# seryrzu/centroFlye

Measured on AMD Instinct MI355X. Metric: long-read bases/sec through rare-k-mer recruit+distance, higher is better.
Workload: dtype u8 bases -> u64 k-mers / u32 indices (integer only)

## Files before the change

### centroflye_amd/csrc/hip/cf_dist.hip

```cpp
#include "cf_common.h"

#include <cstdlib>

void cf_free_edges(cf_ctx* c);
int cf_refresh_unique_count(cf_ctx* ctx);

#define DIST_STAGE_CAP 1024
#define DIST_STACK 112
#define DIST_UNROLL 4
#define DIST_ITEM (64u * DIST_UNROLL)
#define DIST_BM_BITS 65536u
#define DIST_HOT_CAP 2048u
#define DIST_MEMBER_KEYS 8
#define DIST_EDGE_CHUNK 8192ull
#define DIST_OVQ 160u
#define DIST_LDS_HEAD (DIST_BM_BITS / 8 + 128)
#define DIST_CNT_MASK 0x7FFFFFu
#define DIST_SEL_BIT (1ull << 23)

#ifndef cf_ballot
__device__ __forceinline__ unsigned long long cf_ballot(bool p) { return __builtin_amdgcn_ballot_w64(p); }
#endif

struct alignas(16) cf_dist_rec { uint32_t e0; uint32_t len; uint32_t ig; uint32_t nu; };
// ... 138 lines not shown
    const unsigned long long lt = (1ull << lane) - 1ull;
    for (int64_t s0 = wave * (64 * kRounds); s0 < n_kmers; s0 += n_waves * (64 * kRounds)) {
        uint32_t takes = 0, total = 0;
#pragma unroll
        for (int r = 0; r < kRounds; ++r) {
            const int64_t a = s0 + (int64_t)r * 64 + lane;
            const bool take = a < n_kmers && (a % n_parts) == part && pcnt[a] > 0;
            takes |= (uint32_t)take << r;
            total += (uint32_t)__popcll(cf_ballot(take));
        }
        if (total == 0u) continue;
        unsigned long long base = 0;
        if (lane == 0) base = atomicAdd(n_out, (unsigned long long)total);
        base = __shfl(base, 0);
#pragma unroll
        for (int r = 0; r < kRounds; ++r) {
            const bool take = (takes >> r) & 1u;
            const unsigned long long m = cf_ballot(take);
            if (take) {
                const int64_t a = s0 + (int64_t)r * 64 + lane;
                unsigned long long h = 0;
                if (hashed) {
                    const int64_t p0 = post_ptr[a], p1 = post_ptr[a + 1];
                    if (by_second) h = (unsigned long long)(uint32_t)post[p1 - p0 > 1 ? p0 + 1 : p0] & ((1ull << hb) - 1ull);
                    else {
                    h = (unsigned long long)(p1 - p0);
                    for (int64_t p = p0; p < p1; ++p) { h = (h ^ (unsigned long long)(uint32_t)post[p]) * 0x9E3779B97F4A7C15ull; h ^= h >> 29; }
                    h = (h * 0xBF58476D1CE4E5B9ull) >> (64 - hb);
                    }
                }
                keys[base + (unsigned long long)__popcll(m & lt)] = ((unsigned long long)first_unit[a] << (ab + hb)) | (h << ab) | (unsigned long long)a;
            }
            base += (unsigned long long)__popcll(m);
        }
    }
}
__global__ void __launch_bounds__(256)
cf_order_extract_kernel(const unsigned long long* __restrict__ keys, int64_t n, int ab, int32_t* __restrict__ order) {
    const int64_t stride = (int64_t)gridDim.x * blockDim.x;
    for (int64_t i = (int64_t)blockIdx.x * blockDim.x + threadIdx.x; i < n; i += stride) order[i] = (int32_t)(keys[i] & ((1ull << ab) - 1ull));
}

#define DIST_CLASS_CAP 255u
__device__ __forceinline__ bool cf_same_postings(const int64_t* __restrict__ post_ptr, const int32_t* __restrict__ post, uint32_t x, uint32_t y) {
    const int64_t x0 = post_ptr[x], x1 = post_ptr[x + 1], y0 = post_ptr[y], y1 = post_ptr[y + 1];
    if (x1 - x0 != y1 - y0) return false;
    for (int64_t i = 0; i < x1 - x0; ++i) if (post[x0 + i] != post[y0 + i]) return false;
    return true;
}
__global__ void __launch_bounds__(256)
cf_class_mark_kernel(const unsigned long long* __restrict__ keys, int64_t n, int ab, const int64_t* __restrict__ post_ptr, const int32_t* __restrict__ post,
                     const unsigned long long* __restrict__ not_a_set, uint32_t* __restrict__ flags) {
    const unsigned long long rank_mask = (1ull << ab) - 1ull;
    const bool off = *not_a_set != 0ull;
    auto continues = [&](int64_t i) -> bool {
        const unsigned long long k0 = keys[i - 1], k1 = keys[i];
        return (k0 >> ab) == (k1 >> ab) && cf_same_postings(post_ptr, post, (uint32_t)(k0 & rank_mask), (uint32_t)(k1 & rank_mask));
    };
    const int64_t stride = (int64_t)gridDim.x * blockDim.x;
    for (int64_t i = (int64_t)blockIdx.x * blockDim.x + threadIdx.x; i < n; i += stride) {
        if (off) { flags[i] = 1u; continue; }
        if (i > 0 && continues(i)) continue;
        flags[i] = 1u;
        uint32_t run = 1;
        for (int64_t j = i + 1; j < n && continues(j); ++j) {
            if (run == DIST_CLASS_CAP) { flags[j] = 1u; run = 0; }
            ++run;
        }
    }
}
__global__ void __launch_bounds__(256)
cf_class_first_kernel(const uint32_t* __restrict__ flags, const int64_t* __restrict__ cidx, int64_t n, int64_t n_classes, uint32_t* __restrict__ cfirst) {
    const int64_t stride = (int64_t)gridDim.x * blockDim.x;
    for (int64_t i = (int64_t)blockIdx.x * blockDim.x + threadIdx.x; i < n; i += stride) {
        if (flags[i]) cfirst[cidx[i]] = (uint32_t)i;
        if (i == 0) cfirst[n_classes] = (uint32_t)n;
    }
}

#define DIST_GROUP_MAX 32u
__device__ __forceinline__ unsigned long long cf_readlane64(unsigned long long v, int l) {
    return ((unsigned long long)(uint32_t)__builtin_amdgcn_readlane((int)(uint32_t)(v >> 32), l) << 32) | (unsigned long long)(uint32_t)__builtin_amdgcn_readlane((int)(uint32_t)v, l);
}
__global__ void __launch_bounds__(256)
cf_group_mark_kernel(const unsigned long long* __restrict__ keys, int64_t n, int kb, int ab, const int64_t* __restrict__ post_ptr, const int32_t* __restrict__ post,
                     const unsigned long long* __restrict__ not_a_set, uint32_t cap, uint32_t* __restrict__ flags, uint32_t* __restrict__ member_mask, uint32_t* __restrict__ new_mask) {
    const uint32_t lane = threadIdx.x & 63u;
    const int64_t wave = ((int64_t)blockIdx.x * blockDim.x + threadIdx.x) >> 6, n_waves = ((int64_t)gridDim.x * blockDim.x) >> 6;
    const unsigned long long rank_mask = (1ull << ab) - 1ull;
    const bool off = *not_a_set != 0ull;
    for (int64_t c0 = wave * 64; c0 < n; c0 += n_waves * 64) {
        int64_t wb = c0, w_p0 = 0;
        unsigned long long w_fu = ~0ull;
        uint32_t w_len = 0;
        auto load_window = [&](int64_t b) {
            wb = b; w_fu = ~0ull; w_p0 = 0; w_len = 0;
            const int64_t i = b + (int64_t)lane;
            if (i < n) { const unsigned long long k = keys[i]; const uint32_t x = (uint32_t)(k & rank_mask); w_fu = k >> kb; w_p0 = post_ptr[x]; w_len = (uint32_t)(post_ptr[x + 1] - w_p0); }
        };
        load_window(c0);
        const int64_t i_me = c0 + (int64_t)lane;
        if (off) { if (i_me < n) { flags[i_me] = 1u; member_mask[i_me] = 0u; new_mask[i_me] = 0u; } continue; }
        bool head = i_me < n;
        if (head && i_me > 0) head = (keys[i_me - 1] >> kb) != w_fu;
        unsigned long long hm = cf_ballot(head);
        while (hm) {
            const int s = __ffsll((long long)hm) - 1;
            hm &= hm - 1ull;
            if (wb != c0) load_window(c0);
            const unsigned long long fu = cf_readlane64(w_fu, s);
            uint32_t un = 0xFFFFFFFFu, nu = 0, members = 0;
            for (int64_t j = c0 + s; j < n; ++j) {
                if (j - wb == 64) load_window(j);
                const int sl = (int)(j - wb);
                if (cf_readlane64(w_fu, sl) != fu) break;
                const int64_t p0 = (int64_t)cf_readlane64((unsigned long long)w_p0, sl);
                const uint32_t len = (uint32_t)__builtin_amdgcn_readlane((int)w_len, sl);
                if (len > cap) {
                    if (lane == 0u) { flags[j] = 1u; member_mask[j] = 0u; new_mask[j] = 0u; }
                    nu = 0; members = 0;
                    continue;
                }
                const uint32_t L = lane < len ? (uint32_t)post[p0 + lane] : 0xFFFFFFFFu;
                uint32_t mask = 0;
                unsigned long long found = 0;
                for (uint32_t i = 0; i < nu; ++i) {
                    const unsigned long long h = cf_ballot(L == (uint32_t)__builtin_amdgcn_readlane((int)un, (int)i));
                    if (h) { mask |= 1u << i; found |= h; }
                }
                const unsigned long long mine = cf_ballot(lane < len);
                unsigned long long nm = mine & ~found;
                const bool start = members == 0u || members == DIST_CLASS_CAP || nu + (uint32_t)__popcll(nm) > cap;
                if (start) { nu = 0; members = 0; mask = 0; nm = mine; }
                const uint32_t fresh = (uint32_t)nm;
                while (nm) {
                    const int t = __ffsll((long long)nm) - 1;
                    nm &= nm - 1ull;
                    const uint32_t x = (uint32_t)__builtin_amdgcn_readlane((int)L, t);
                    if (lane == nu) un = x;
                    mask |= 1u << nu;
                    ++nu;
                }
                ++members;
                if (lane == 0u) { if (start) flags[j] = 1u; member_mask[j] = mask; new_mask[j] = fresh; }
            }
        }
    }
}
__global__ void __launch_bounds__(256)
cf_group_fill_kernel(const int32_t* __restrict__ order, const uint32_t* __restrict__ gfirst, int64_t n_groups, const int64_t* __restrict__ post_ptr, const int32_t* __restrict__ post,
                     const unsigned long long* __restrict__ not_a_set, uint32_t cap, const uint32_t* __restrict__ new_mask, const uint32_t* __restrict__ member_mask,
                     int32_t* __restrict__ upost, uint32_t* __restrict__ ulen, unsigned long long* __restrict__ diag, unsigned long long* __restrict__ err) {
    const bool off = *not_a_set != 0ull;
    unsigned long long dg_u = 0, dg_c = 0;
    const int64_t stride = (int64_t)gridDim.x * blockDim.x;
    for (int64_t g = (int64_t)blockIdx.x * blockDim.x + threadIdx.x; g < n_groups; g += stride) {
        const uint32_t f = gfirst[g], e = gfirst[g + 1];
        bool counting = off;
        if (e - f == 1u) { const int32_t x = order[f]; counting = counting || (uint32_t)(post_ptr[x + 1] - post_ptr[x]) > cap; }
        uint32_t k = 0;
        if (!counting)
            for (uint32_t j = f; j < e; ++j) {
                uint32_t nm = new_mask[j];
                if (!nm) continue;
                const int64_t p0 = post_ptr[order[j]];
                while (nm) {
                    const int t = __ffs((int)nm) - 1;
                    nm &= nm - 1u;
                    if (k < DIST_GROUP_MAX) upost[(size_t)DIST_GROUP_MAX * (size_t)g + k] = post[p0 + t];
                    ++k;
                }
            }
        if (k > DIST_GROUP_MAX) { atomicOr(err, 4ull); k = DIST_GROUP_MAX; }
        ulen[g] = counting ? 0x80000000u : k;
        dg_u += k;
#if defined(CF_DIST_DIAG_COUNT)
        for (uint32_t j = f; j < e; ++j) {
            bool seen = false;
            for (uint32_t q = f; q < j && !seen; ++q) seen = member_mask[q] == member_mask[j];
            dg_c += (unsigned long long)!seen;
        }
#endif
    }
#if defined(CF_DIST_DIAG_COUNT)
    for (int d = 32; d >= 1; d >>= 1) { dg_u += __shfl_down(dg_u, (unsigned)d); dg_c += __shfl_down(dg_c, (unsigned)d); }
    if ((threadIdx.x & 63) == 0 && dg_c) { atomicAdd(diag, dg_u); atomicAdd(diag + 1, dg_c); }
#else
    (void)diag; (void)dg_u; (void)dg_c; (void)member_mask;
#endif
}
__global__ void __launch_bounds__(256)
cf_member_emissions_kernel(const int32_t* __restrict__ order, int64_t n_order, const int64_t* __restrict__ post_ptr, const int32_t* __restrict__ post,
                           const cf_dist_rec* __restrict__ urange, const int32_t* __restrict__ rend, int32_t min_d, int32_t max_d,
                           unsigned long long* __restrict__ entries_out, unsigned long long* __restrict__ self_out) {
    unsigned long long ent = 0, self = 0;
    const int64_t stride = (int64_t)gridDim.x * blockDim.x;
    for (int64_t i = (int64_t)blockIdx.x * blockDim.x + threadIdx.x; i < n_order; i += stride) {
        const int32_t x = order[i];
        const int64_t p0 = post_ptr[x], p1 = post_ptr[x + 1];
        int32_t u = p0 < p1 ? post[p0] : 0;
        for (int64_t p = p0; p < p1; ++p) {
            ent += urange[u].len;
            const int32_t u_next = p + 1 < p1 ? post[p + 1] : 0x7FFFFFFF;
            if (u_next < rend[u]) {
                for (int64_t q = p + 1; q < p1; ++q) {
                    const int32_t v = post[q];
                    if (v >= rend[u] || v - u > max_d) break;
                    self += (unsigned long long)(v - u >= min_d);
                }
            }
            u = u_next;
        }
    }
    for (int d = 32; d >= 1; d >>= 1) { ent += __shfl_down(ent, (unsigned)d); self += __shfl_down(self, (unsigned)d); }
    if ((threadIdx.x & 63) == 0) {
        if (ent) atomicAdd(entries_out, ent);
        if (self) atomicAdd(self_out, self);
    }
}

struct alignas(8) cf_dist_item { uint32_t e, m; };
#ifndef CF_DIST_ITEMS_BLOCKED
#define CF_DIST_ITEMS_BLOCKED 0
#endif
struct alignas(16) cf_dist_head { uint32_t a, n_items; unsigned long long ibase; uint32_t n_entries, n_useful, n_members, first_member; };

struct cf_dist_args {
    const int64_t* post_ptr;
    const int32_t* post;
    const int64_t* cloud_ptr;
    const int32_t* entries;
    const int32_t* unit_rend;
    const int32_t* unit_rbeg;
    const cf_dist_rec* urange;
    const uint16_t* entry_i;
    const uint8_t* entry_i8;
    uint32_t reg_shift;
    const uint32_t* packed;
    int64_t n_kmers;
    int32_t part, n_parts;
    int32_t min_d, max_d;
    uint32_t min_cov;
    double thr;
    uint32_t thr_num, thr_den;
    int32_t slots;
    uint32_t fill_limit;
    uint32_t est_limit;
    int32_t sketch;
    uint32_t sk_counters, sk_shift, sk_mask;
    uint32_t sk_fbits, sk_fsh, sk_wshift, sk_fmask, sk_guard, sk_bytes;
    const cf_dist_head* heads;
    const cf_dist_item* items;
    uint32_t stage_cap;
    uint32_t filter_once;
    uint32_t hot_cap;
    uint32_t hot_entries;
    uint32_t* edges;
    unsigned long long edge_cap;
    const uint32_t* member_mask;
    const int32_t* order;
    int64_t n_order;
    unsigned long long edge_chunk;
    unsigned long long* holes;
    unsigned long long* counters;
    uint32_t* unique_bits;
};

typedef uint32_t cf_raw4 __attribute__((ext_vector_type(4)));
struct __attribute__((packed, aligned(4))) cf_run4 { uint32_t x, y, z, w; };
__device__ __forceinline__ void cf_load_packed4(const cf_dist_args& A, uint32_t s_e, uint32_t l4, uint32_t& x, uint32_t& y, uint32_t& z, uint32_t& w) {
#if !defined(CF_NO_BUFFER_LOAD)
    const __amdgpu_buffer_rsrc_t rs = __builtin_amdgcn_make_buffer_rsrc((void*)A.packed, 0, (int)0xFFFFFFFFu, 0x00020000);
    const cf_raw4 v = __builtin_amdgcn_raw_buffer_load_b128(rs, (int)(l4 * 4u), (int)(s_e << 2), 0);
    x = v.x; y = v.y; z = v.z; w = v.w;
#else
    const uint32_t* p = A.packed + s_e;
    const cf_run4 r = *(const cf_run4*)(p + l4);
    x = r.x; y = r.y; z = r.z; w = r.w;
#endif
}

struct alignas(16) cf_u64x2 { unsigned long long x, y; };
struct alignas(16) cf_u32x4 { uint32_t x, y, z, w; };

template <int DB>
struct cf_tab_wide_t {
    static constexpr uint32_t kCntBits = 31 - DB, kCntMask = (1u << kCntBits) - 1u, kDMask = (1u << DB) - 1u, kDShift = 32 - DB;
    static constexpr uint32_t kSlotBytes = 8, kPerBucket = 4;
    static constexpr bool kMaskTab = false;
    struct bucket { cf_u64x2 lo, hi; };
    struct raw { uint32_t b, i; };
    typedef unsigned long long qitem;
    static __device__ __forceinline__ qitem q_make(uint32_t b, uint32_t dd, uint32_t bk) { return ((unsigned long long)b << 32) | ((unsigned long long)dd << kDShift) | bk; }
    static __device__ __forceinline__ void q_take(qitem q, uint32_t n_buckets, uint32_t& b, uint32_t& dd, uint32_t& bk) { b = (uint32_t)(q >> 32); dd = ((uint32_t)q >> kDShift) & kDMask; bk = (uint32_t)q & ((1u << kDShift) - 1u); }
    __device__ __forceinline__ qitem q_of(uint32_t b, uint32_t dd, uint32_t n_buckets) const { return q_make(b, dd, home(hash(b), n_buckets)); }
    static __device__ __forceinline__ uint32_t next(uint32_t bk, uint32_t, uint32_t n_buckets) { return bk + 1 == n_buckets ? 0u : bk + 1; }
    __device__ __forceinline__ void configure(const cf_dist_args&, uint32_t) {}
    unsigned long long* tab;
    __device__ __forceinline__ void init(unsigned char* lds, uint32_t) { tab = (unsigned long long*)lds; }
    __device__ __forceinline__ void clear(uint32_t slots, uint32_t t, uint32_t nt) const {
        const cf_u64x2 z{0ull, 0ull};
// ... 1959 lines not shown
        unsigned long long partner_units = 0;
        for (int64_t r = min_n; r < max_n; ++r) {
            const int64_t nu = v_h_unit_ptr[(size_t)r + 1] - v_h_unit_ptr[(size_t)r];
            const int64_t span = (int64_t)max_d - min_d_eff + 1;
            if (nu <= min_d_eff || span <= 0) continue;
            const int64_t full = std::max<int64_t>(0, nu - max_d);
            const int64_t tail = nu - min_d_eff - full;
            partner_units += (unsigned long long)(full * span) + (unsigned long long)(tail > 0 ? tail * (tail + 1) / 2 : 0);
        }
        const double cloud = (double)(e1 - e0) / (double)(u1 - u0), post_per_unit = (double)n_post / (double)(u1 - u0);
        per_first = (double)partner_units * cloud * post_per_unit / (double)std::max<int64_t>(1, (K - part + n_parts - 1) / n_parts);
    }
    const bool groups = groups_fit && per_first <= 32768.0;
    const uint32_t slot_bytes = groups ? cf_tab_mask<8>::kSlotBytes : (narrow || region) ? cf_tab_narrow::kSlotBytes : cf_tab_wide::kSlotBytes;
    int wgs = ctx->dist_wgs, block = ctx->dist_block;
    if (wgs == 0) wgs = (block > 512 || per_first > 32768.0) ? 1 : 2;
    if (block == 0) block = wgs == 1 ? 1024 : 512;
    const size_t qitem_bytes = narrow ? sizeof(cf_tab_narrow::qitem) : sizeof(cf_tab_wide::qitem);
    const size_t lds_fixed = DIST_LDS_HEAD + (size_t)(2 * DIST_STACK) * 4 + DIST_STAGE_CAP * 2 + 16 + (size_t)(block / 64) * (DIST_QSTRIDE + DIST_OVQ) * qitem_bytes + DIST_HOT_CAP * 2
                             + (groups ? (((size_t)(block / 64) * (DIST_QSTRIDE + DIST_OVQ) + 15) & ~(size_t)15) : 0);
    const int64_t budget8 = ((int64_t)160 * 1024 / wgs - (int64_t)lds_fixed) / 8;
    if (budget8 < 256) return cf_fail(ctx, -22, "cf_dist_edges: dist_wgs leaves no LDS for the table");
    if (ctx->dist_slots > budget8) return cf_fail(ctx, -22, "cf_dist_edges: dist_slots does not fit the 160 KiB LDS next to the work lists");
    const int64_t slots8 = ctx->dist_slots ? ctx->dist_slots : budget8;
    A.slots = (int32_t)((slots8 * 8 / slot_bytes) & ~(region ? (int64_t)(32 << reg_shift) - 1 : 7ll));
    if (groups) {
        A.slots = (int32_t)((slots8 * 8 / cf_tab_mask<8>::kSlotBytes) & ~7ll);
        while (A.slots > 8 && (int64_t)A.slots * cf_tab_mask<8>::kSlotBytes + cf_tab_mask<8>::extra_bytes((uint32_t)A.slots) > slots8 * 8) A.slots -= 8;
    }
    const size_t tab_extra = groups ? cf_tab_mask<8>::extra_bytes((uint32_t)A.slots) : 0;
    if (A.slots >= 0xFFFF) return cf_fail(ctx, -22, "cf_dist_edges: more than 65534 table slots (16-bit slot indices; 0xFFFF marks an unused entry of the hot list)");
    A.fill_limit = (uint32_t)((int64_t)A.slots * ctx->dist_fill_pct / 100);
    {
        const int64_t slack = (int64_t)(block / 64) * 2 * 128;
        if (slack * 4 <= (int64_t)A.slots) A.fill_limit = (uint32_t)std::min<int64_t>(A.fill_limit, (int64_t)A.slots - slack);
    }
    A.est_limit = (uint32_t)((int64_t)A.fill_limit * 100 / ctx->dist_est_pct);
    A.counters = d_cnt; A.unique_bits = ctx->d_unique_bits;
    const size_t lds = (size_t)A.slots * slot_bytes + tab_extra + lds_fixed;
    A.sketch = (ctx->dist_sketch && min_cov >= 2 && min_cov <= 200) ? 1 : 0;
    A.sk_shift = 32; A.sk_counters = 1;
    const size_t sk_room = (size_t)A.slots * slot_bytes + DIST_STAGE_CAP * 2 + 16 + (size_t)(block / 64) * (DIST_QSTRIDE + DIST_OVQ) * qitem_bytes + 2 * DIST_STACK * 4 + DIST_HOT_CAP * 2;
    while (A.sk_shift > 8 && (size_t)A.sk_counters * 2 <= sk_room) { A.sk_counters *= 2; --A.sk_shift; }
    if (A.sk_counters < 16) A.sketch = 0;
    A.sk_bytes = A.sk_counters;
    const bool sk4 = A.sketch && min_cov <= 9 && ctx->dist_sketch_bits != 8 && A.sk_shift > 9;
    if (sk4) { A.sk_counters *= 2; --A.sk_shift; A.sk_fbits = 4; A.sk_fsh = 2; A.sk_wshift = 3; A.sk_fmask = 15; A.sk_guard = 12; }
    else { A.sk_fbits = 8; A.sk_fsh = 3; A.sk_wshift = 2; A.sk_fmask = 255; A.sk_guard = 0x7FFFFFFFu; }
    A.sk_mask = A.sk_counters - 1u;
    const int per_cu = std::max(1, std::min((int)((160 * 1024) / lds), 2048 / block));
    const int64_t n_a_alloc = (K > part) ? (K - part + n_parts - 1) / n_parts : 0;
    CF_TRY(tmp.get(&d_okeys, (size_t)n_a_alloc, "order keys"));
    CF_TRY(tmp.get(&d_otmp, (size_t)n_a_alloc, "order scratch"));
    CF_TRY(tmp.get(&d_order, (size_t)n_a_alloc, "order"));
    int ab = 1, ub = 1;
    while (ab < 32 && ((int64_t)1 << ab) < K) ++ab;
    while (ub < 32 && ((int64_t)1 << ub) < std::max<int64_t>(U, 2)) ++ub;
    const bool classes = ctx->dist_classes && by_sort;
    const int hb = classes ? std::min(ctx->dist_class_bits, 64 - ab - ub) : 0;
    int64_t n_heads = 0;
    uint32_t *d_cflag = nullptr, *d_cfirst = nullptr, *d_ulen = nullptr, *d_mmask = nullptr, *d_newm = nullptr;
    int32_t* d_upost = nullptr;
    if (K) {
        hipLaunchKernelGGL(cf_order_keys_kernel, dim3((unsigned)cf_grid_for(K, 256, max_blocks)), dim3(256), 0, ctx->stream,
                           (const uint32_t*)d_pcnt, (const uint32_t*)d_first, K, (int)part, (int)n_parts, ab, d_okeys, d_cnt + 6,
                           hb, (const int64_t*)d_post_ptr, (const int32_t*)d_post, (const unsigned long long*)(d_cnt + 144), groups ? 1 : 0);
        unsigned long long h_n = 0;
        CF_HIP(hipMemcpy(&h_n, d_cnt + 6, 8, hipMemcpyDeviceToHost));
        n_order = (int64_t)h_n;
        CF_TRY(cf_radix_sort_u64(ctx, d_okeys, d_otmp, n_order, ab + hb + ub));
        if (n_order)
            hipLaunchKernelGGL(cf_order_extract_kernel, dim3((unsigned)cf_grid_for(n_order, 256, max_blocks)), dim3(256), 0, ctx->stream,
                               (const unsigned long long*)d_okeys, n_order, ab, d_order);
    }
    n_heads = n_order;
    if (classes && n_order) {
        const unsigned g_cls = (unsigned)cf_grid_for(n_order, 256, max_blocks);
        int64_t* d_cidx = (int64_t*)d_otmp;
        CF_TRY(tmp.get(&d_cflag, (size_t)n_order + 1, "class flags"));
        CF_TRY(tmp.get(&d_cfirst, (size_t)n_order + 1, "class starts"));
        CF_HIP(hipMemsetAsync(d_cflag, 0, (size_t)(n_order + 1) * 4, ctx->stream));
        if (groups) { CF_TRY(tmp.get(&d_mmask, (size_t)n_order + 1, "member masks")); CF_TRY(tmp.get(&d_newm, (size_t)n_order + 1, "members' new postings")); }
        if (groups)
            hipLaunchKernelGGL(cf_group_mark_kernel, dim3(g_cls), dim3(256), 0, ctx->stream, (const unsigned long long*)d_okeys, n_order, ab + hb, ab,
                               (const int64_t*)d_post_ptr, (const int32_t*)d_post, (const unsigned long long*)(d_cnt + 144), (uint32_t)ctx->dist_group_cap, d_cflag, d_mmask, d_newm);
        else
        hipLaunchKernelGGL(cf_class_mark_kernel, dim3(g_cls), dim3(256), 0, ctx->stream, (const unsigned long long*)d_okeys, n_order, ab,
                           (const int64_t*)d_post_ptr, (const int32_t*)d_post, (const unsigned long long*)(d_cnt + 144), d_cflag);
        CF_TRY(cf_scan_exclusive_u32_to_i64(ctx, d_cflag, d_cidx, n_order, &n_heads));
        hipLaunchKernelGGL(cf_class_first_kernel, dim3(g_cls), dim3(256), 0, ctx->stream, (const uint32_t*)d_cflag, (const int64_t*)d_cidx, n_order, n_heads, d_cfirst);
        if (groups) {
            CF_TRY(tmp.get(&d_upost, (size_t)n_heads * DIST_GROUP_MAX + 1, "group unions"));
            CF_TRY(tmp.get(&d_ulen, (size_t)n_heads + 1, "group union sizes"));
            hipLaunchKernelGGL(cf_group_fill_kernel, dim3((unsigned)cf_grid_for(n_heads, 256, max_blocks)), dim3(256), 0, ctx->stream, (const int32_t*)d_order, (const uint32_t*)d_cfirst, n_heads,
                               (const int64_t*)d_post_ptr, (const int32_t*)d_post, (const unsigned long long*)(d_cnt + 144), (uint32_t)ctx->dist_group_cap, (const uint32_t*)d_newm, (const uint32_t*)d_mmask,
                               d_upost, d_ulen, d_cnt + 148, d_cnt + 4);
            hipLaunchKernelGGL(cf_member_emissions_kernel, dim3(g_cls), dim3(256), 0, ctx->stream, (const int32_t*)d_order, n_order, (const int64_t*)d_post_ptr, (const int32_t*)d_post,
                               (const cf_dist_rec*)d_urange, (const int32_t*)d_rend, min_d_eff, max_d, d_cnt + 1, d_cnt + 3);
        }
        CF_KERNEL_CHECK("the class kernels");
    }
    A.order = d_order; A.n_order = n_heads; A.member_mask = d_mmask;
    if (n_heads) {
        const uint32_t nw = (uint32_t)block / 64u;
        const int g_items = cf_grid_for(n_heads * 16, 256, max_blocks);
        CF_TRY(tmp.get(&d_icnt, (size_t)n_heads + 1, "item counts"));
        CF_TRY(tmp.get(&d_ialloc, (size_t)n_heads + 1, "item slots"));
        CF_TRY(tmp.get(&d_ibase, (size_t)n_heads + 1, "item bases"));
        CF_TRY(tmp.get(&d_heads, (size_t)n_heads, "first k-mer heads"));
        hipLaunchKernelGGL(groups ? cf_items_count_kernel<true> : cf_items_count_kernel<false>, dim3((unsigned)g_items), dim3(256), 0, ctx->stream, (const int32_t*)d_order, n_heads, (const int64_t*)d_post_ptr,
                           (const int32_t*)d_post, (const cf_dist_rec*)d_urange, (const int32_t*)d_rbeg, min_d_eff, max_d, nw, by_sort ? 1 : 0, d_icnt, d_ialloc, d_cnt + 3,
                           (const uint32_t*)d_cfirst, (const int32_t*)d_upost, (const uint32_t*)d_ulen);
        CF_TRY(cf_scan_exclusive_u32_to_i64(ctx, d_ialloc, d_ibase, n_heads, &n_item_slots));
        CF_TRY(tmp.get(&d_items, (size_t)n_item_slots + 64, "item records"));
        hipLaunchKernelGGL(groups ? cf_items_fill_kernel<true> : cf_items_fill_kernel<false>, dim3((unsigned)g_items), dim3(256), 0, ctx->stream, (const int32_t*)d_order, n_heads, (const int64_t*)d_post_ptr,
                           (const int32_t*)d_post, (const cf_dist_rec*)d_urange, nw, (const uint32_t*)d_icnt, (const int64_t*)d_ibase, d_heads, d_items,
                           v_cloud_ptr, region26 ? 1 : 0, U, min_d_eff, max_d, min_cov, (ctx->dist_sketch_tail && A.sketch) ? 1 : 0,
                           (const unsigned long long*)(d_cnt + 144), d_cnt + 145, (const uint32_t*)d_cfirst, (const int32_t*)d_upost, (const uint32_t*)d_ulen);
    }
    A.heads = d_heads; A.items = d_items;
    const int64_t n_a = n_heads;
    const int grid = (int)std::max<int64_t>(1, std::min<int64_t>(n_a, (int64_t)std::max(1, ctx->n_cu) * per_cu));
    CF_KERNEL_CHECK("the work-list kernels");
    CF_HIP(hipEventRecord(ctx->ev2, ctx->stream));
#define CF_DIST_KERN(CLS) (region26 ? cf_dist_kernel<cf_tab_region26, CLS> : region ? cf_dist_kernel<cf_tab_region, CLS> : !narrow ? (wide16 ? cf_dist_kernel<cf_tab_wide16, CLS> : cf_dist_kernel<cf_tab_wide, CLS>) \
                               : narrow_db == 8 ? cf_dist_kernel<cf_tab_narrow_t<8>, CLS> : narrow_db == 7 ? cf_dist_kernel<cf_tab_narrow_t<7>, CLS>                                               \
                               : narrow_db == 6 ? cf_dist_kernel<cf_tab_narrow_t<6>, CLS> : cf_dist_kernel<cf_tab_narrow_t<5>, CLS>)
    void (*kern)(cf_dist_args) = classes ? CF_DIST_KERN(true) : CF_DIST_KERN(false);
#if CF_DIST_HAS_GROUPS
    if (groups) kern = narrow_db == 8 ? cf_dist_kernel<cf_tab_mask<8>, true> : narrow_db == 7 ? cf_dist_kernel<cf_tab_mask<7>, true> : narrow_db == 6 ? cf_dist_kernel<cf_tab_mask<6>, true> : cf_dist_kernel<cf_tab_mask<5>, true>;
#endif
#undef CF_DIST_KERN
    CF_HIP(hipFuncSetAttribute((const void*)kern, hipFuncAttributeMaxDynamicSharedMemorySize, (int)lds));
    {
        A.edge_chunk = ctx->dist_edge_chunk > 0 ? (unsigned long long)ctx->dist_edge_chunk : DIST_EDGE_CHUNK;
        const int64_t rows = edge_cap > 0 ? edge_cap + (int64_t)grid * (int64_t)A.edge_chunk : 0;
        CF_TRY(cf_alloc_t(ctx, &ctx->d_edges, (size_t)rows * 4, "edges"));
        ctx->edge_cap = rows;
        A.edges = ctx->d_edges; A.edge_cap = (unsigned long long)rows;
    }
    CF_TRY(tmp.get(&d_holes, 2 * ((size_t)grid + 1), "edge holes"));
    A.holes = d_holes;
    CF_HIP(hipMemsetAsync(d_cnt + 6, 0, 16, ctx->stream));
    if (n_a > 0 && max_d >= min_d_eff && n_post > 0) {
        hipLaunchKernelGGL(kern, dim3((unsigned)grid), dim3((unsigned)block), lds, ctx->stream, A);
        CF_KERNEL_CHECK("cf_dist_kernel");
    }
    CF_HIP(hipEventRecord(ctx->ev3, ctx->stream));
    CF_HIP(hipMemcpyAsync(h_cnt, d_cnt, 64, hipMemcpyDeviceToHost, ctx->stream));
    CF_HIP(hipEventRecord(ctx->ev1, ctx->stream));
    CF_HIP(hipEventSynchronize(ctx->ev1));
#if defined(CF_DIST_DIAG_COUNT)
    {
        unsigned long long st[8];
        if (hipMemcpy(st, d_cnt + 8, 64, hipMemcpyDeviceToHost) == hipSuccess)
            std::fprintf(stderr, "[cf_dist diag] parked-insert loop trips=%llu overflow calls=%llu parked inserts run=%llu drains=%llu inserts drained=%llu cycles(sum over waves): parked runs=%llu drains=%llu table sweeps=%llu; waves=%d passes=%llu\n", st[0], st[1], st[2], st[3], st[4], st[5], st[6], st[7], grid * (block / 64), h_cnt[5]);
        unsigned long long su[4], up[2] = {0, 0};
        const bool have_up = groups && hipMemcpy(up, d_cnt + 148, 16, hipMemcpyDeviceToHost) == hipSuccess;
        if (hipMemcpy(su, d_cnt + 144, 32, hipMemcpyDeviceToHost) == hipSuccess)
            std::fprintf(stderr, "[cf_dist diag] sketch items=%llu of items=%llu (rows are sets=%d) classes=%lld members=%lld entries swept=%llu of %llu per member\n", su[1], su[2], su[0] ? 0 : 1, have_up ? (long long)up[1] : (long long)n_heads, (long long)n_order, su[3], h_cnt[1]);
        unsigned long long mf[5];
        if (hipMemcpy(mf, d_cnt + 152, 40, hipMemcpyDeviceToHost) == hipSuccess)
            std::fprintf(stderr, "[cf_dist diag] member filter: n_hot=%llu n_hot x members=%llu eval_slot calls with total_of=%llu buckets read in total_of=%llu slots with more keys than registers=%llu\n", mf[0], mf[1], mf[2], mf[3], mf[4]);
        if (have_up)
            std::fprintf(stderr, "[cf_dist diag] groups=%lld members=%lld union postings=%llu slots=%d split groups=%llu\n", (long long)n_heads, (long long)n_order, up[0], (int)A.slots, h_cnt[2]);
    }
#endif
#if defined(CF_DIST_STAMPS)
    {
        unsigned long long st[8];
        if (hipMemcpy(st, d_cnt + 8, 64, hipMemcpyDeviceToHost) == hipSuccess)
            std::fprintf(stderr, "[cf_dist stamps] pop=%llu prologue=%llu sketch=%llu clear=%llu stream=%llu filter=%llu write=%llu sweep_end_wait=%llu (shader cycles summed over %d workgroups; passes=%llu)\n",
                         st[0], st[1], st[6], st[2], st[3], st[4], st[5], st[7], grid, h_cnt[5]);
    }
#endif
    if (h_cnt[4] & 4ull) return cf_fail(ctx, -5, "cf_dist_edges: internal error, a group's union has more postings than its mask has bits");
    if (h_cnt[4] & 2ull) return cf_fail(ctx, -5, "cf_dist_edges: the kernel's dynamic LDS does not begin at address 0");
    if (h_cnt[4]) return cf_fail(ctx, -34, "cf_dist_edges: (b,d) table could not be partitioned far enough");
    {
        const unsigned long long a_cap = std::min<unsigned long long>(h_cnt[0], A.edge_cap);
        std::vector<unsigned long long> hh(2 * (size_t)h_cnt[7]);
// ... 59 lines not shown
```

Before: 4.847 billion.

## Fuse member emissions into group-walk kernel with LDS-staged postings and team fill

Replaces the group mark kernel with a walk kernel that stages each window's posting lists into per-wave LDS rows using 8-lane teams. The entry and self-distance counts come from those staged rows in the same pass, so the separate member-emissions kernel and its second read of postings are gone. The member loop now reads postings from LDS with a prefetch, and per-member outputs are buffered in lanes and stored coalesced. The fill kernel moves from one thread per group to 8-lane teams with a prefix-sum scatter. In exchange it adds LDS use that may lower occupancy, more register pressure, and a more complex control flow with correctness risk (caps clamped to 32).

```diff
diff --git a/centroflye_amd/csrc/hip/cf_dist.hip b/centroflye_amd/csrc/hip/cf_dist.hip
--- a/centroflye_amd/csrc/hip/cf_dist.hip
+++ b/centroflye_amd/csrc/hip/cf_dist.hip
@@ -244,23 +244,121 @@
 __device__ __forceinline__ unsigned long long cf_readlane64(unsigned long long v, int l) {
     return ((unsigned long long)(uint32_t)__builtin_amdgcn_readlane((int)(uint32_t)(v >> 32), l) << 32) | (unsigned long long)(uint32_t)__builtin_amdgcn_readlane((int)(uint32_t)v, l);
 }
+#define DIST_WALK_ROW 33u
+#define DIST_WALK_LDS(block) ((size_t)((block) / 64) * 64 * DIST_WALK_ROW * 4)
 __global__ void __launch_bounds__(256)
-cf_group_mark_kernel(const unsigned long long* __restrict__ keys, int64_t n, int kb, int ab, const int64_t* __restrict__ post_ptr, const int32_t* __restrict__ post,
-                     const unsigned long long* __restrict__ not_a_set, uint32_t cap, uint32_t* __restrict__ flags, uint32_t* __restrict__ member_mask, uint32_t* __restrict__ new_mask) {
+cf_group_walk_kernel(const unsigned long long* __restrict__ keys, int64_t n, int kb, int ab, const int64_t* __restrict__ post_ptr, const int32_t* __restrict__ post,
+                     const unsigned long long* __restrict__ not_a_set, uint32_t cap, const cf_dist_rec* __restrict__ urange, const int32_t* __restrict__ rend, int32_t min_d, int32_t max_d,
+                     uint32_t* __restrict__ flags, uint32_t* __restrict__ member_mask, uint32_t* __restrict__ new_mask,
+                     unsigned long long* __restrict__ entries_out, unsigned long long* __restrict__ self_out) {
     const uint32_t lane = threadIdx.x & 63u;
+    uint32_t* const rows = (uint32_t*)cf_lds + (size_t)(threadIdx.x >> 6) * (64u * DIST_WALK_ROW);
     const int64_t wave = ((int64_t)blockIdx.x * blockDim.x + threadIdx.x) >> 6, n_waves = ((int64_t)gridDim.x * blockDim.x) >> 6;
     const unsigned long long rank_mask = (1ull << ab) - 1ull;
     const bool off = *not_a_set != 0ull;
+    if (cap > DIST_GROUP_MAX) cap = DIST_GROUP_MAX;
+    unsigned long long ent = 0, self = 0;
     for (int64_t c0 = wave * 64; c0 < n; c0 += n_waves * 64) {
         int64_t wb = c0, w_p0 = 0;
         unsigned long long w_fu = ~0ull;
-        uint32_t w_len = 0;
-        auto load_window = [&](int64_t b) {
+        uint32_t w_len = 0, o_mask = 0, o_new = 0;
+        bool o_start = false, o_done = false;
+        auto flush = [&]() {
+            if (o_done) { const int64_t i = wb + (int64_t)lane; flags[i] = o_start ? 1u : 0u; member_mask[i] = o_mask; new_mask[i] = o_new; }
+            o_done = false;
+        };
+        auto load_window = [&](int64_t b, bool all, bool own, unsigned long long fu) {
+            flush();
             wb = b; w_fu = ~0ull; w_p0 = 0; w_len = 0;
             const int64_t i = b + (int64_t)lane;
-            if (i < n) { const unsigned long long k = keys[i]; const uint32_t x = (uint32_t)(k & rank_mask); w_fu = k >> kb; w_p0 = post_ptr[x]; w_len = (uint32_t)(post_ptr[x + 1] - w_p0); }
+            if (i < n) {
+                const unsigned long long k = keys[i];
+                w_fu = k >> kb;
+                if (all || w_fu == fu) { const uint32_t x = (uint32_t)(k & rank_mask); w_p0 = post_ptr[x]; w_len = (uint32_t)(post_ptr[x + 1] - w_p0); }
+            }
+            const uint32_t len_l = w_len <= DIST_GROUP_MAX ? w_len : 0u;
+            const uint32_t tl = lane & 7u, team = lane >> 3;
+            unsigned long long adj_m = 0;
+            int64_t t_p0[8];
+            uint32_t t_len[8];
+            int32_t t_u[8], t_r[8];
+            uint32_t t_el[8], t_ig[8];
+            __builtin_amdgcn_wave_barrier();
+#pragma unroll
+            for (int r = 0; r < 8; ++r) {
+                const int m = r * 8 + (int)team;
+                t_p0[r] = (int64_t)__shfl((long long)w_p0, m);
+                t_len[r] = __shfl(len_l, m);
+                t_u[r] = post[t_p0[r] + (int64_t)(tl < t_len[r] ? tl : 0u)];
+            }
+            if (own) {
+#pragma unroll
+                for (int r = 0; r < 8; ++r) { t_el[r] = urange[t_u[r]].len; t_ig[r] = urange[t_u[r]].ig; }
+            }
+#pragma unroll
+            for (int r = 0; r < 8; ++r) {
+                const uint32_t m = (uint32_t)r * 8u + team;
+                const bool on = tl < t_len[r];
+                if (on) rows[m * DIST_WALK_ROW + tl] = (uint32_t)t_u[r];
+                t_r[r] = -1;
+                if (own) {
+                    if (on) { ent += t_el[r]; t_r[r] = t_u[r] - (int32_t)t_ig[r]; }
+                    const int32_t prev = __shfl_up(t_r[r], 1u, 8);
+                    if (on && tl > 0u && t_r[r] == prev) adj_m |= 1ull << m;
+                }
+            }
+#pragma unroll
+            for (int r = 0; r < 8; ++r) {
+                const uint32_t m = (uint32_t)r * 8u + team;
+                int32_t r_carry = own ? __shfl(t_r[r], 7, 8) : -1;
+                for (uint32_t k0 = 8u; cf_ballot(k0 < t_len[r]) != 0ull; k0 += 8u) {
+                    const uint32_t k = k0 + tl;
+                    const bool on = k < t_len[r];
+                    const int32_t u = post[t_p0[r] + (int64_t)(on ? k : 0u)];
+                    if (on) rows[m * DIST_WALK_ROW + k] = (uint32_t)u;
+                    if (own) {
+                        int32_t rr = -1;
+                        if (on) { ent += urange[u].len; rr = u - (int32_t)urange[u].ig; }
+                        int32_t prev = __shfl_up(rr, 1u, 8);
+                        if (tl == 0u) prev = r_carry;
+                        if (on && rr == prev) adj_m |= 1ull << m;
+                        r_carry = __shfl(rr, 7, 8);
+                    }
+                }
+            }
+            bool adj = false;
+            if (own && cf_ballot(adj_m != 0ull) != 0ull) {
+                for (int d = 32; d >= 1; d >>= 1) adj_m |= (unsigned long long)__shfl_xor((long long)adj_m, d);
+                adj = (adj_m >> lane) & 1ull;
+            }
+            __builtin_amdgcn_wave_barrier();
+            if (!own) return;
+            if (adj)
+                for (uint32_t p = 0; p + 1u < len_l; ++p) {
+                    const int32_t up = (int32_t)rows[lane * DIST_WALK_ROW + p], re = rend[up];
+                    for (uint32_t q = p + 1u; q < len_l; ++q) {
+                        const int32_t v = (int32_t)rows[lane * DIST_WALK_ROW + q];
+                        if (v >= re || v - up > max_d) break;
+                        self += (unsigned long long)(v - up >= min_d);
+                    }
+                }
+            unsigned long long lm = cf_ballot(w_len > DIST_GROUP_MAX);
+            while (lm) {
+                const int sl = __ffsll((long long)lm) - 1;
+                lm &= lm - 1ull;
+                const int64_t p0 = (int64_t)cf_readlane64((unsigned long long)w_p0, sl), p1 = p0 + (int64_t)(uint32_t)__builtin_amdgcn_readlane((int)w_len, sl);
+                for (int64_t p = p0 + (int64_t)lane; p < p1; p += 64) {
+                    const int32_t up = post[p], re = rend[up];
+                    ent += urange[up].len;
+                    for (int64_t q = p + 1; q < p1; ++q) {
+                        const int32_t v = post[q];
+                        if (v >= re || v - up > max_d) break;
+                        self += (unsigned long long)(v - up >= min_d);
+                    }
+                }
+            }
         };
-        load_window(c0);
+        load_window(c0, true, true, 0ull);
         const int64_t i_me = c0 + (int64_t)lane;
         if (off) { if (i_me < n) { flags[i_me] = 1u; member_mask[i_me] = 0u; new_mask[i_me] = 0u; } continue; }
         bool head = i_me < n;
@@ -269,70 +367,97 @@
         while (hm) {
             const int s = __ffsll((long long)hm) - 1;
             hm &= hm - 1ull;
-            if (wb != c0) load_window(c0);
+            if (wb != c0) load_window(c0, true, false, 0ull);
             const unsigned long long fu = cf_readlane64(w_fu, s);
-            uint32_t un = 0xFFFFFFFFu, nu = 0, members = 0;
+            uint32_t un = 0xFFFFFFFEu, nu = 0, members = 0;
+            uint32_t L_next = rows[(uint32_t)s * DIST_WALK_ROW + (lane & 31u)];
             for (int64_t j = c0 + s; j < n; ++j) {
-                if (j - wb == 64) load_window(j);
+                if (j - wb == 64) { load_window(j, false, false, fu); L_next = rows[lane & 31u]; }
                 const int sl = (int)(j - wb);
                 if (cf_readlane64(w_fu, sl) != fu) break;
-                const int64_t p0 = (int64_t)cf_readlane64((unsigned long long)w_p0, sl);
                 const uint32_t len = (uint32_t)__builtin_amdgcn_readlane((int)w_len, sl);
-                if (len > cap) {
-                    if (lane == 0u) { flags[j] = 1u; member_mask[j] = 0u; new_mask[j] = 0u; }
-                    nu = 0; members = 0;
-                    continue;
+                const uint32_t L = lane < len ? L_next : 0xFFFFFFFFu;
+                L_next = rows[(uint32_t)min(sl + 1, 63) * DIST_WALK_ROW + (lane & 31u)];
+                uint32_t mask = 0, fresh = 0;
+                bool start = true;
+                if (len > cap) { nu = 0; members = 0; }
+                else {
+                    uint32_t found = 0;
+                    if (nu)
+                        for (uint32_t t0 = 0; t0 < len; t0 += 8u) {
+#pragma unroll
+                            for (uint32_t q = 0; q < 8u; ++q) {
+                                const unsigned long long h = cf_ballot(un == (uint32_t)__builtin_amdgcn_readlane((int)L, (int)(t0 + q)));
+                                mask |= (uint32_t)h;
+                                found |= (uint32_t)(h != 0ull) << (t0 + q);
+                            }
+                        }
+                    const uint32_t mine = (uint32_t)((1ull << len) - 1ull);
+                    uint32_t nm = mine & ~found;
+                    start = members == 0u || members == DIST_CLASS_CAP || nu + (uint32_t)__popc(nm) > cap;
+                    if (start) { nu = 0; members = 0; mask = 0; nm = mine; un = 0xFFFFFFFEu; }
+                    fresh = nm;
+                    while (nm) {
+                        const int t = __ffs((int)nm) - 1;
+                        nm &= nm - 1u;
+                        const uint32_t x = (uint32_t)__builtin_amdgcn_readlane((int)L, t);
+                        if (lane == nu) un = x;
+                        mask |= 1u << nu;
+                        ++nu;
+                    }
+                    ++members;
                 }
-                const uint32_t L = lane < len ? (uint32_t)post[p0 + lane] : 0xFFFFFFFFu;
-                uint32_t mask = 0;
-                unsigned long long found = 0;
-                for (uint32_t i = 0; i < nu; ++i) {
-                    const unsigned long long h = cf_ballot(L == (uint32_t)__builtin_amdgcn_readlane((int)un, (int)i));
-                    if (h) { mask |= 1u << i; found |= h; }
-                }
-                const unsigned long long mine = cf_ballot(lane < len);
-                unsigned long long nm = mine & ~found;
-                const bool start = members == 0u || members == DIST_CLASS_CAP || nu + (uint32_t)__popcll(nm) > cap;
-                if (start) { nu = 0; members = 0; mask = 0; nm = mine; }
-                const uint32_t fresh = (uint32_t)nm;
-                while (nm) {
-                    const int t = __ffsll((long long)nm) - 1;
-                    nm &= nm - 1ull;
-                    const uint32_t x = (uint32_t)__builtin_amdgcn_readlane((int)L, t);
-                    if (lane == nu) un = x;
-                    mask |= 1u << nu;
-                    ++nu;
-                }
-                ++members;
-                if (lane == 0u) { if (start) flags[j] = 1u; member_mask[j] = mask; new_mask[j] = fresh; }
-            }
-        }
-    }
-}
+                if (lane == (uint32_t)sl) { o_start = start; o_mask = mask; o_new = fresh; o_done = true; }
+            }
+        }
+        flush();
+    }
+    for (int d = 32; d >= 1; d >>= 1) { ent += __shfl_down(ent, (unsigned)d); self += __shfl_down(self, (unsigned)d); }
+    if (lane == 0u) {
+        if (ent) atomicAdd(entries_out, ent);
+        if (self) atomicAdd(self_out, self);
+    }
+}
+#define DIST_FILL_TEAM 8
 __global__ void __launch_bounds__(256)
 cf_group_fill_kernel(const int32_t* __restrict__ order, const uint32_t* __restrict__ gfirst, int64_t n_groups, const int64_t* __restrict__ post_ptr, const int32_t* __restrict__ post,
                      const unsigned long long* __restrict__ not_a_set, uint32_t cap, const uint32_t* __restrict__ new_mask, const uint32_t* __restrict__ member_mask,
                      int32_t* __restrict__ upost, uint32_t* __restrict__ ulen, unsigned long long* __restrict__ diag, unsigned long long* __restrict__ err) {
     const bool off = *not_a_set != 0ull;
     unsigned long long dg_u = 0, dg_c = 0;
-    const int64_t stride = (int64_t)gridDim.x * blockDim.x;
-    for (int64_t g = (int64_t)blockIdx.x * blockDim.x + threadIdx.x; g < n_groups; g += stride) {
-        const uint32_t f = gfirst[g], e = gfirst[g + 1];
+    constexpr uint32_t T = DIST_FILL_TEAM;
+    const uint32_t tl = threadIdx.x & (T - 1u);
+    const int64_t team = ((int64_t)blockIdx.x * blockDim.x + threadIdx.x) / T, n_teams = ((int64_t)gridDim.x * blockDim.x) / T;
+    for (int64_t g0 = 0; g0 < n_groups; g0 += n_teams) {
+        const int64_t g = g0 + team;
+        const bool on = g < n_groups;
+        uint32_t f = 0, e = 0;
+        if (on) { f = gfirst[g]; e = gfirst[g + 1]; }
         bool counting = off;
-        if (e - f == 1u) { const int32_t x = order[f]; counting = counting || (uint32_t)(post_ptr[x + 1] - post_ptr[x]) > cap; }
+        if (on && e - f == 1u) { const int32_t x = order[f]; counting = counting || (uint32_t)(post_ptr[x + 1] - post_ptr[x]) > cap; }
+        const uint32_t n_mem = (on && !counting) ? e - f : 0u;
+        uint32_t n_max = n_mem;
+        for (uint32_t d = T; d < 64u; d <<= 1) n_max = max(n_max, __shfl_xor(n_max, (int)d));
         uint32_t k = 0;
-        if (!counting)
-            for (uint32_t j = f; j < e; ++j) {
-                uint32_t nm = new_mask[j];
-                if (!nm) continue;
+        for (uint32_t b = 0; b < n_max; b += T) {
+            const uint32_t j = f + b + tl;
+            uint32_t nm = b + tl < n_mem ? new_mask[j] : 0u;
+            const uint32_t c = (uint32_t)__popc(nm);
+            uint32_t incl = c;
+            for (uint32_t d = 1; d < T; d <<= 1) { const uint32_t t = __shfl_up(incl, d, (int)T); if (tl >= d) incl += t; }
+            uint32_t at = k + incl - c;
+            if (nm) {
                 const int64_t p0 = post_ptr[order[j]];
                 while (nm) {
                     const int t = __ffs((int)nm) - 1;
                     nm &= nm - 1u;
-                    if (k < DIST_GROUP_MAX) upost[(size_t)DIST_GROUP_MAX * (size_t)g + k] = post[p0 + t];
-                    ++k;
+                    if (at < DIST_GROUP_MAX) upost[(size_t)DIST_GROUP_MAX * (size_t)g + at] = post[p0 + t];
+                    ++at;
                 }
             }
+            k += __shfl(incl, (int)T - 1, (int)T);
+        }
+        if (!on || tl != 0u) continue;
         if (k > DIST_GROUP_MAX) { atomicOr(err, 4ull); k = DIST_GROUP_MAX; }
         ulen[g] = counting ? 0x80000000u : k;
         dg_u += k;
@@ -350,35 +475,6 @@
 #else
     (void)diag; (void)dg_u; (void)dg_c; (void)member_mask;
 #endif
-}
-__global__ void __launch_bounds__(256)
-cf_member_emissions_kernel(const int32_t* __restrict__ order, int64_t n_order, const int64_t* __restrict__ post_ptr, const int32_t* __restrict__ post,
-                           const cf_dist_rec* __restrict__ urange, const int32_t* __restrict__ rend, int32_t min_d, int32_t max_d,
-                           unsigned long long* __restrict__ entries_out, unsigned long long* __restrict__ self_out) {
-    unsigned long long ent = 0, self = 0;
-    const int64_t stride = (int64_t)gridDim.x * blockDim.x;
-    for (int64_t i = (int64_t)blockIdx.x * blockDim.x + threadIdx.x; i < n_order; i += stride) {
-        const int32_t x = order[i];
-        const int64_t p0 = post_ptr[x], p1 = post_ptr[x + 1];
-        int32_t u = p0 < p1 ? post[p0] : 0;
-        for (int64_t p = p0; p < p1; ++p) {
-            ent += urange[u].len;
-            const int32_t u_next = p + 1 < p1 ? post[p + 1] : 0x7FFFFFFF;
-            if (u_next < rend[u]) {
-                for (int64_t q = p + 1; q < p1; ++q) {
-                    const int32_t v = post[q];
-                    if (v >= rend[u] || v - u > max_d) break;
-                    self += (unsigned long long)(v - u >= min_d);
-                }
-            }
-            u = u_next;
-        }
-    }
-    for (int d = 32; d >= 1; d >>= 1) { ent += __shfl_down(ent, (unsigned)d); self += __shfl_down(self, (unsigned)d); }
-    if ((threadIdx.x & 63) == 0) {
-        if (ent) atomicAdd(entries_out, ent);
-        if (self) atomicAdd(self_out, self);
-    }
 }
 
 struct alignas(8) cf_dist_item { uint32_t e, m; };
@@ -2504,8 +2600,9 @@
         CF_HIP(hipMemsetAsync(d_cflag, 0, (size_t)(n_order + 1) * 4, ctx->stream));
         if (groups) { CF_TRY(tmp.get(&d_mmask, (size_t)n_order + 1, "member masks")); CF_TRY(tmp.get(&d_newm, (size_t)n_order + 1, "members' new postings")); }
         if (groups)
-            hipLaunchKernelGGL(cf_group_mark_kernel, dim3(g_cls), dim3(256), 0, ctx->stream, (const unsigned long long*)d_okeys, n_order, ab + hb, ab,
-                               (const int64_t*)d_post_ptr, (const int32_t*)d_post, (const unsigned long long*)(d_cnt + 144), (uint32_t)ctx->dist_group_cap, d_cflag, d_mmask, d_newm);
+            hipLaunchKernelGGL(cf_group_walk_kernel, dim3(g_cls), dim3(256), DIST_WALK_LDS(256), ctx->stream, (const unsigned long long*)d_okeys, n_order, ab + hb, ab,
+                               (const int64_t*)d_post_ptr, (const int32_t*)d_post, (const unsigned long long*)(d_cnt + 144), (uint32_t)ctx->dist_group_cap,
+                               (const cf_dist_rec*)d_urange, (const int32_t*)d_rend, min_d_eff, max_d, d_cflag, d_mmask, d_newm, d_cnt + 1, d_cnt + 3);
         else
         hipLaunchKernelGGL(cf_class_mark_kernel, dim3(g_cls), dim3(256), 0, ctx->stream, (const unsigned long long*)d_okeys, n_order, ab,
                            (const int64_t*)d_post_ptr, (const int32_t*)d_post, (const unsigned long long*)(d_cnt + 144), d_cflag);
@@ -2514,11 +2611,9 @@
         if (groups) {
             CF_TRY(tmp.get(&d_upost, (size_t)n_heads * DIST_GROUP_MAX + 1, "group unions"));
             CF_TRY(tmp.get(&d_ulen, (size_t)n_heads + 1, "group union sizes"));
-            hipLaunchKernelGGL(cf_group_fill_kernel, dim3((unsigned)cf_grid_for(n_heads, 256, max_blocks)), dim3(256), 0, ctx->stream, (const int32_t*)d_order, (const uint32_t*)d_cfirst, n_heads,
+            hipLaunchKernelGGL(cf_group_fill_kernel, dim3((unsigned)cf_grid_for(n_heads * DIST_FILL_TEAM, 256, max_blocks)), dim3(256), 0, ctx->stream, (const int32_t*)d_order, (const uint32_t*)d_cfirst, n_heads,
                                (const int64_t*)d_post_ptr, (const int32_t*)d_post, (const unsigned long long*)(d_cnt + 144), (uint32_t)ctx->dist_group_cap, (const uint32_t*)d_newm, (const uint32_t*)d_mmask,
                                d_upost, d_ulen, d_cnt + 148, d_cnt + 4);
-            hipLaunchKernelGGL(cf_member_emissions_kernel, dim3(g_cls), dim3(256), 0, ctx->stream, (const int32_t*)d_order, n_order, (const int64_t*)d_post_ptr, (const int32_t*)d_post,
-                               (const cf_dist_rec*)d_urange, (const int32_t*)d_rend, min_d_eff, max_d, d_cnt + 1, d_cnt + 3);
         }
         CF_KERNEL_CHECK("the class kernels");
     }
```

Result: faster. 4.918 billion (median of 6 runs) (+1.5%).
